# medhini/audio-video-textures

Measured on AMD Instinct MI355X. Metric: clip-windows/sec encoded + N×N transition build, N=4096; HBM GB/s achieved, higher is better.
Workload: dtype f16x3

## Files before the change

audio-video-textures_amd/csrc/conv_x3.hip:

```cpp
#include <stdlib.h>

#include <type_traits>

#include "avt_common.h"
#include "conv_args.h"
#include "split_planes.h"

#ifdef AVT_CONV_STAMP
#define AVT_STAMP_FN avt_debug_stamps_x3
namespace {
#include "../../tools/diag/conv_stamp.h"
}
#ifndef AVT_DBG_CONST
#define AVT_DBG_CONST 0
#endif
#define DBG_SKIP(bit) (((AVT_DBG_CONST) & (bit)) != 0)
#ifdef AVT_STAMP_EPI
#define KSTAMP(i) STAMP(0)
#define EPI_STAMP(i) STAMP(i)
#else
#define KSTAMP(i) STAMP(i)
#define EPI_STAMP(i)
#endif
#else
// ... 762 lines not shown
            }
          }
          float* of = reinterpret_cast<float*>(a.out) + o;
          typedef float f32x4n __attribute__((ext_vector_type(4)));
          __builtin_nontemporal_store(f32x4n{x[0], x[1], x[2], x[3]}, reinterpret_cast<f32x4n*>(of));
          __builtin_nontemporal_store(f32x4n{x[4], x[5], x[6], x[7]}, reinterpret_cast<f32x4n*>(of + 4));
        } else {
          uint4 oh, ol;
          avt::split8<F16>(x, oh, ol);
          *reinterpret_cast<uint4*>(a.out + o) = oh;
          *reinterpret_cast<uint4*>(a.out_lo + o) = ol;
        }
      }
    }
    EPI_STAMP(3);
    __syncthreads();
    EPI_STAMP(4);
  }
  if constexpr (IO32) {
    if (a.stat_part) {
      float* red = reinterpret_cast<float*>(lds);
      const int tr = tid / CPR, cc = tid % CPR;
#pragma unroll
      for (int e = 0; e < 8; ++e) {
        red[(tr * 2 + 0) * BN + cc * 8 + e] = st_s[e];
        red[(tr * 2 + 1) * BN + cc * 8 + e] = st_q[e];
      }
      __syncthreads();
      stat_fold_store<BN, NTHR>(a, red, NTHR / CPR, tm, n0, tid);
    }
  }
  STAMP_END();
}

template <bool F16, bool IO32 = false, bool OUT32 = IO32>
int launch_x3_xl(ConvArgs& a, hipStream_t st) {
  if (a.stat_part) a.stat_tpg = (a.stat_mg + 255) / 256;
  const int tiles_m = a.stat_part ? a.stat_groups * a.stat_tpg : (a.M + 255) / 256;
  a.tiles_n = (a.Cout + 255) / 256;
  a.nblk = tiles_m * a.tiles_n;
  constexpr int lds_max = 2 * 4 * 256 * 64 + kMaxTabSteps * 64 + 2 * 256 * 4;
  const int lds_bytes = lds_max;
  a.cf_ofs = lds_max - 2 * 256 * 4;
  static const hipError_t e = hipFuncSetAttribute(reinterpret_cast<const void*>(conv_x3_xl_kernel<F16, IO32, OUT32>),
                                                  hipFuncAttributeMaxDynamicSharedMemorySize, lds_max);
  if (e != hipSuccess) {
    avt::set_error("avt_conv3d_igemm_x3: hipFuncSetAttribute(%d B LDS): %s", lds_max, hipGetErrorString(e));
    return AVT_ERR_LAUNCH;
  }
  hipLaunchKernelGGL((conv_x3_xl_kernel<F16, IO32, OUT32>), dim3((unsigned)a.nblk), dim3(512), lds_bytes, st, a);
  return avt::check_launch("avt_conv3d_igemm_x3");
}

template <int BM, int BN, int WTM, bool F16, bool IO32 = false, bool BST = false>
int launch_x3(ConvArgs& a, hipStream_t st) {
  if (a.stat_part) a.stat_tpg = (a.stat_mg + BM - 1) / BM;
  const int tiles_m = a.stat_part ? a.stat_groups * a.stat_tpg : (a.M + BM - 1) / BM;
  a.tiles_n = (a.Cout + BN - 1) / BN;
  a.nblk = tiles_m * a.tiles_n;
  constexpr int epi_bytes = BM * (BN * 4 + 16);
  constexpr int opnd_max = 2 * (BM + BN) * LSTR + kMaxTabSteps * 64;
  constexpr int lds_max = (opnd_max > epi_bytes ? opnd_max : epi_bytes) + 2 * BN * 4;
  const int tab_bytes = (a.nk <= kMaxTabSteps ? a.nk : 0) * 64;
  int lds_bytes = 2 * (BM + BN) * LSTR + tab_bytes;
  if (lds_bytes < epi_bytes) lds_bytes = epi_bytes;
  a.cf_ofs = lds_bytes;
  lds_bytes += 2 * BN * 4;
  static const hipError_t e = hipFuncSetAttribute(reinterpret_cast<const void*>(conv_x3_kernel<BM, BN, WTM, F16, IO32, BST>),
                                                  hipFuncAttributeMaxDynamicSharedMemorySize, lds_max);
  if (e != hipSuccess) {
    avt::set_error("avt_conv3d_igemm_x3: hipFuncSetAttribute(%d B LDS): %s", lds_max, hipGetErrorString(e));
    return AVT_ERR_LAUNCH;
  }
  hipLaunchKernelGGL((conv_x3_kernel<BM, BN, WTM, F16, IO32, BST>), dim3((unsigned)a.nblk), dim3(256), lds_bytes, st, a);
  return avt::check_launch("avt_conv3d_igemm_x3");
}

}

extern "C" int avt_conv3d_igemm_x3_xl_picked(int cout, int k, int m) {
  return (cout % 256 == 0 && k >= 256 && k <= kMaxTabSteps * 64 && m >= 256 * 64) ? 1 : 0;
}

static int igemm_x3_impl(const void* in_hi, const void* in_lo, const void* wt_hi, const void* wt_lo,
                         const float* bias, const void* res_hi, const void* res_lo, void* out_hi, void* out_lo,
                         const int32_t* ktab, int batch, int t, int h, int w, int cin, int cout, int kt, int kh,
                         int kw, int st, int sh, int sw, int pt, int ph, int pw, int to, int ho, int wo, int ldi,
                         int ldo, int ldr, int relu, int out_row_stride, int out_h, int out_w, int plane_dtype,
                         const float* wscale, void* stream, int wblk) {
  AVT_REQUIRE(plane_dtype == AVT_X3_BF16 || plane_dtype == AVT_X3_F16, "avt_conv3d_igemm_x3: plane_dtype must be 0 (bf16) or 1 (fp16)");
  AVT_REQUIRE(!wscale || avt::aligned16(wscale), "avt_conv3d_igemm_x3: wscale must be 16-byte aligned");
  AVT_REQUIRE(in_lo && wt_lo && out_lo && (!res_hi == !res_lo), "avt_conv3d_igemm_x3: every tensor needs both planes");
  AVT_REQUIRE(avt::aligned16(in_lo) && avt::aligned16(wt_lo) && avt::aligned16(out_lo) && (!res_lo || avt::aligned16(res_lo)),
              "avt_conv3d_igemm_x3: pointers must be 16-byte aligned");
  ConvArgs a;
  const int rc = conv_args_fill(a, "avt_conv3d_igemm_x3", in_hi, wt_hi, bias, res_hi, out_hi, ktab, batch, t, h, w, cin, cout,
                                kt, kh, kw, st, sh, sw, pt, ph, pw, to, ho, wo, ldi, ldo, ldr, relu, out_row_stride, out_h,
                                out_w);
  if (rc != AVT_OK) return rc;
  a.in_lo = static_cast<const uint16_t*>(in_lo);
  a.wt_lo = static_cast<const uint16_t*>(wt_lo);
  a.res_lo = static_cast<const uint16_t*>(res_lo);
  a.out_lo = static_cast<uint16_t*>(out_lo);
  a.wscale = wscale;
  a.wfrag = nullptr;
  a.nup = 0;
  a.wblk = wblk;
  hipStream_t s = static_cast<hipStream_t>(stream);
  AVT_REQUIRE(!wblk || (avt_conv3d_igemm_x3_xl_picked(cout, a.K, a.M) && a.K % 32 == 0),
              "avt_conv3d_igemm_x3_wblk: K-blocked weights are the 256 x 256 tile's (avt_conv3d_igemm_x3_xl_picked, K %% 32 == 0)");
  if (avt_conv3d_igemm_x3_xl_picked(cout, a.K, a.M))
    return plane_dtype == AVT_X3_F16 ? launch_x3_xl<true>(a, s) : launch_x3_xl<false>(a, s);
  if (plane_dtype == AVT_X3_F16) {
    if (cout <= 32) return launch_x3<128, 32, 32, true>(a, s);
    if (cout <= 64) return launch_x3<128, 64, 64, true>(a, s);
    return launch_x3<128, 128, 64, true>(a, s);
  }
  if (cout <= 32) return launch_x3<128, 32, 32, false>(a, s);
  if (cout <= 64) return launch_x3<128, 64, 64, false>(a, s);
  return launch_x3<128, 128, 64, false>(a, s);
}

extern "C" int avt_conv3d_igemm_x3(const void* in_hi, const void* in_lo, const void* wt_hi, const void* wt_lo,
                                   const float* bias, const void* res_hi, const void* res_lo, void* out_hi, void* out_lo,
                                   const int32_t* ktab, int batch, int t, int h, int w, int cin, int cout, int kt, int kh,
                                   int kw, int st, int sh, int sw, int pt, int ph, int pw, int to, int ho, int wo, int ldi,
                                   int ldo, int ldr, int relu, int out_row_stride, int out_h, int out_w, int plane_dtype,
                                   const float* wscale, void* stream) {
  return igemm_x3_impl(in_hi, in_lo, wt_hi, wt_lo, bias, res_hi, res_lo, out_hi, out_lo, ktab, batch, t, h, w, cin, cout, kt, kh, kw,
                       st, sh, sw, pt, ph, pw, to, ho, wo, ldi, ldo, ldr, relu, out_row_stride, out_h, out_w, plane_dtype, wscale,
                       stream, 0);
}

extern "C" int avt_conv3d_igemm_x3_wblk(const void* in_hi, const void* in_lo, const void* wt_hi, const void* wt_lo,
                                        const float* bias, const void* res_hi, const void* res_lo, void* out_hi, void* out_lo,
                                        const int32_t* ktab, int batch, int t, int h, int w, int cin, int cout, int kt, int kh,
                                        int kw, int st, int sh, int sw, int pt, int ph, int pw, int to, int ho, int wo, int ldi,
                                        int ldo, int ldr, int relu, int out_row_stride, int out_h, int out_w, int plane_dtype,
                                        const float* wscale, void* stream) {
  return igemm_x3_impl(in_hi, in_lo, wt_hi, wt_lo, bias, res_hi, res_lo, out_hi, out_lo, ktab, batch, t, h, w, cin, cout, kt, kh, kw,
                       st, sh, sw, pt, ph, pw, to, ho, wo, ldi, ldo, ldr, relu, out_row_stride, out_h, out_w, plane_dtype, wscale,
                       stream, 1);
}

extern "C" int avt_gemm_nt_x3_f32out(const void* a_hi, const void* a_lo, int lda, const void* b_hi, const void* b_lo, float* out, int64_t ldo,
                                     int m, int n, int k, float divisor, const int32_t* ktab, int plane_dtype, void* stream) {
  AVT_REQUIRE(plane_dtype == AVT_X3_BF16 || plane_dtype == AVT_X3_F16, "avt_gemm_nt_x3_f32out: plane_dtype must be 0 (bf16) or 1 (fp16)");
  AVT_REQUIRE(a_lo && b_lo && avt::aligned16(a_lo) && avt::aligned16(b_lo) && divisor != 0.0f, "avt_gemm_nt_x3_f32out: both planes, divisor != 0");
  AVT_REQUIRE(m > 0 && n % 256 == 0 && k % 32 == 0 && k >= 256 && k <= kMaxTabSteps * 64 && ldo >= n && ldo % 4 == 0 && ldo < (1ll << 31),
              "avt_gemm_nt_x3_f32out: n %% 256 == 0, 256 <= k <= %d in multiples of 32 (got m %d n %d k %d)", kMaxTabSteps * 64, m, n, k);
  ConvArgs a;
  const int rc = conv_args_fill(a, "avt_gemm_nt_x3_f32out", a_hi, b_hi, nullptr, nullptr, out, ktab, 1, 1, 1, m, k, n, 1, 1, 1, 1, 1, 1, 0, 0, 0,
                                0, 0, 0, lda, 8 * (int)((ldo + 7) / 8), 0, 0, 1, 0, 0);
  if (rc != AVT_OK) return rc;
  a.ldo = (int)ldo;
  a.in_lo = static_cast<const uint16_t*>(a_lo);
  a.wt_lo = static_cast<const uint16_t*>(b_lo);
  a.res_lo = nullptr;
  a.out_lo = nullptr;
  a.wscale = nullptr;
  a.wfrag = nullptr;
  a.nup = 0;
  a.wblk = 0;
  a.odiv = divisor;
  hipStream_t s = static_cast<hipStream_t>(stream);
  return plane_dtype == AVT_X3_F16 ? launch_x3_xl<true, false, true>(a, s) : launch_x3_xl<false, false, true>(a, s);
}

static int g_io32_small = 1;
static int io32_tile_rows(int cout, int k, int64_t m) {
  if (k % 32 == 0 && m < (1ll << 31) && avt_conv3d_igemm_x3_xl_picked(cout, k, (int)m) && m >= 256 * 256) return 256;
  if (g_io32_small && cout > 64 && ((m + 127) / 128) * ((cout + 127) / 128) < 512) return 64;
  return 128;
}

extern "C" int avt_conv_x3_set_small_tile(int on) {
  const int was = g_io32_small;
  g_io32_small = on ? 1 : 0;
  return was;
}

static int igemm_x3_f32_impl(const float* in, const void* wt_hi, const void* wt_lo, const float* wscale, const float* add,
                             float* out, const int32_t* ktab, int batch, int t, int h, int w, int cin, int cout, int kt, int kh,
                             int kw, int st, int sh, int sw, int pt, int ph, int pw, int to, int ho, int wo, int ldi, int ldo, int lda,
                             int out_row_stride, int out_h, int out_w, int plane_dtype, void* stream, double* stat_part = nullptr,
                             int stat_groups = 0, int stat_c = 0, const ConvArgs* bst = nullptr) {
  AVT_REQUIRE(plane_dtype == AVT_X3_BF16 || plane_dtype == AVT_X3_F16, "avt_conv3d_igemm_x3_f32: plane_dtype must be 0 (bf16) or 1 (fp16)");
  AVT_REQUIRE(wt_lo && avt::aligned16(wt_lo) && (!wscale || avt::aligned16(wscale)), "avt_conv3d_igemm_x3_f32: weight planes / wscale NULL or unaligned");
  AVT_REQUIRE((int64_t)batch * t * h * w * ldi < (1ll << 30) - 64, "avt_conv3d_igemm_x3_f32: input too large for 32-bit byte offsets");
  ConvArgs a;
  const int rc = conv_args_fill(a, "avt_conv3d_igemm_x3_f32", in, wt_hi, nullptr, add, out, ktab, batch, t, h, w, cin, cout, kt, kh, kw,
                                st, sh, sw, pt, ph, pw, to, ho, wo, ldi, ldo, add ? lda : 0, 0, out_row_stride, out_h, out_w);
  if (rc != AVT_OK) return rc;
  a.in_bytes *= 2u;
  a.in_lo = nullptr;
  a.wt_lo = static_cast<const uint16_t*>(wt_lo);
  a.res_lo = nullptr;
  a.out_lo = nullptr;
  a.wscale = wscale;
  a.wfrag = nullptr;
  a.nup = 0;
  a.wblk = 0;
  if (stat_part) {
// ... 99 lines not shown
```

audio-video-textures_amd/fused_slowfast.py:

```python
import torch
import torch.nn as nn

from . import ops
from ._lib import AvtError


_FUSE_BLOCK = 1
_C33 = 1
_CHAIN = 1
_CHAIN_MAXN = 512
_FUSE_KCAT = 1
_XB = 1
_FUSE_SCAT = 1
_FUSE_TCHUNK = 0
_FUSE_BLOCK_X3 = 1
_FUSE_TCHUNK_X3 = 0
_CHAIN_X3 = 1
_WBLK_X3 = 1
_STEM_FM_X3 = 1
_C33_X3 = 1
_RES2_X3 = 1
_PW_X3 = 1
_STEM_LDS = 1
_STEM_POOL = 1
_PW_X3_SKIP = {(512, 128), (320, 128)}
_LATERAL_X3 = {(32, 64)}
_STEM_MERGE = 1
_KW1_CAP = 32

PROFILER = None


class Act:

    __slots__ = ("buf", "dims", "c0", "C", "lo")

    def __init__(self, buf, dims, c0=0, C=None, lo=None):
        self.buf, self.dims, self.c0, self.lo = buf, dims, c0, lo
        self.C = buf.shape[1] - c0 if C is None else C

    @property
    def ptr(self):
        return self.buf.data_ptr() + 2 * self.c0

    @property
    def ptrs(self):
        return (self.buf.data_ptr() + 2 * self.c0, self.lo.data_ptr() + 2 * self.c0)

    @property
    def ld(self):
        return self.buf.shape[1]

    def float(self, plane_dtype=None):
        if self.lo is None:
            return self.buf[:, self.c0 : self.c0 + self.C].float()
        dt = torch.float16 if plane_dtype == ops.X3_F16 else torch.bfloat16
        sl = slice(self.c0, self.c0 + self.C)
        return self.buf.view(dt)[:, sl].float() + self.lo.view(dt)[:, sl].float()


def new_act(m, c, dims, device, x3=False):
    buf = torch.empty((m, c), dtype=torch.bfloat16, device=device)
    return Act(buf, dims, lo=torch.empty_like(buf) if x3 else None)


def split_planes(w, plane_dtype):
    w = w.detach().float()
    dt = torch.float16 if plane_dtype == ops.X3_F16 else torch.bfloat16
    hi = w.to(dt)
    lo = (w - hi.float()).to(dt)
    return hi.view(torch.bfloat16).contiguous(), lo.view(torch.bfloat16).contiguous()


def fold_bn(conv, bn):
    w = conv.weight.detach().float()
    if bn is not None:
        scale = bn.weight.detach().float() / torch.sqrt(bn.running_var.detach().float() + bn.eps)
        bias = bn.bias.detach().float() - bn.running_mean.detach().float() * scale
        w = w * scale.view(-1, 1, 1, 1, 1)
    else:
        bias = conv.bias.detach().float() if conv.bias is not None else torch.zeros(w.shape[0])
    return w, bias


def group_weights_w(w, g):
    cout, cin, kt, kh, kw = w.shape
    r = kw // 2
    rg = -(-r // g)
    kwg = 1 + 2 * rg
    wg = torch.zeros((g, cout, g, cin, kt, kh, kwg))
    for po in range(g):
        for dg in range(kwg):
            for pi in range(g):
                dw = g * (dg - rg) + pi - po + r
                if 0 <= dw < kw:
                    wg[po, :, pi, :, :, :, dg] = w[:, :, :, :, dw]
    return wg.reshape(g * cout, g * cin, kt, kh, kwg), rg
# ... 614 lines not shown
                return self._chain(m, self.c.cin, self.c, sc, chain, m.dims, y=out, x2=x2)
            return self.c(m, out=out, res=sc, relu=True)
        if (self.fused is not None and out is None and x.c0 == 0 and x.ld == x.C and
                ops.bottleneck_fused_supported(x.C, x.dims[3])):
            b, t, h, w = x.dims
            y = Act(torch.empty((b * t * h * w, x.C), dtype=torch.bfloat16, device=self.dev), x.dims)

            def launch():
                ops.bottleneck_fused(x.ptr, y.ptr, self.fused, b, t, h, w, x.C, tchunk=_FUSE_TCHUNK or (16 if w >= 56 else 32))

            if PROFILER is None:
                launch()
            else:
                m = b * t * h * w
                fl = m * (self.a.alg_flops_per_row + self.b.alg_flops_per_row + self.c.alg_flops_per_row)
                PROFILER("bottleneck_kernel", launch, fl, 2.0 * (2 * m * x.C))
            return y
        if (self.fused_first is not None and out is None and x.c0 == 0 and x.ld == x.C and
                ops.bottleneck_first_supported(x.C, self.c.cout, x.dims[3]) and x.dims[2] % self.b.stride[1] == 0):
            b, t, h, w = x.dims
            st = self.b.stride[1]
            od = (b, t, h // st, w // st)
            mo = od[0] * od[1] * od[2] * od[3]
            y = Act(torch.empty((mo, self.c.cout), dtype=torch.bfloat16, device=self.dev), od)

            def launch():
                ops.bottleneck_first(x.ptr, y.ptr, self.fused_first, b, t, h, w, x.C, self.c.cout,
                                     tchunk=_FUSE_TCHUNK or (16 if w >= 56 else 32))

            if PROFILER is None:
                launch()
            else:
                m = b * t * h * w
                fl = (m * self.a.alg_flops_per_row +
                      mo * (self.b.alg_flops_per_row + self.c.alg_flops_per_row + self.b1.alg_flops_per_row))
                PROFILER("bottleneck_kernel", launch, fl, 2.0 * (m * x.C + mo * self.c.cout))
            return y
        sc = self.b1(x) if self.b1 is not None else x
        return self.c(self._b(self.a(x)), out=out, res=sc, relu=True)


class _BlockX3:

    def __init__(self, blk, device, x3):
        self.b1 = FusedConv(blk.branch1, blk.branch1_bn, False, device, x3=x3) if hasattr(blk, "branch1") else None
        t = blk.branch2
        self.a = FusedConv(t.a, t.a_bn, True, device, x3=x3)
        self.b = FusedConv(t.b, t.b_bn, True, device, x3=x3)
        self.c = FusedConv(t.c, t.c_bn, True, device, x3=x3)
        self.x3, self.dev = x3, device
        self.fused = None
        shape_ok = (self.a.kernel == (3, 1, 1) and self.b.kernel == (1, 3, 3) and self.c.kernel == (1, 1, 1) and
                    self.a.stride == (1, 1, 1) and self.a.cout <= 32)
        s1 = self.b.stride == (1, 1, 1)
        ident = s1 and self.b1 is None and self.c.cout == self.a.cin and self.c.cout in (32, 64, 128)
        first8 = (s1 and self.b1 is not None and self.a.cin == 8 and self.c.cout == 32 and self.b1.kernel == (1, 1, 1) and
                  self.b1.stride == (1, 1, 1))
        strided = (self.b1 is not None and self.b.stride == (1, 2, 2) and self.b1.stride == (1, 2, 2) and
                   self.b1.kernel == (1, 1, 1) and self.a.cin in (32, 64) and self.c.cout == 2 * self.a.cin)
        self.st = 2 if strided else 1
        if _FUSE_BLOCK_X3 and shape_ok and (ident or first8 or strided):
            (wa, ba), (wb, bb), (wc, bc) = self.a._folded, self.b._folded, self.c._folded
            self.fused = pack_bottleneck_x3(wa, ba, wb, bb, wc, bc, x3, device,
                                            shortcut=self.b1._folded if (first8 or strided) else None)
        self.c33 = None
        if (_C33_X3 and self.fused is None and self.b.kernel == (1, 3, 3) and self.b.stride == (1, 1, 1) and
                self.b._folded is not None and ops.conv33_x3_supported(self.b.cin, self.b.cout)):
            self.c33 = pack_c33_x3(self.b._folded[0], self.b._folded[1], x3, device)
        self.res2 = None
        if (_RES2_X3 and x3 == ops.X3_F16 and self.fused is None and self.b1 is None and self.a.kernel == (1, 1, 1) and
                self.a.stride == (1, 1, 1) and self.b.kernel == (1, 3, 3) and self.b.stride == (1, 1, 1) and self.c.kernel == (1, 1, 1) and
                self.c.stride == (1, 1, 1) and self.a.cin == self.c.cout and all(v._folded is not None for v in (self.a, self.b, self.c)) and
                ops.res2_x3_supported(self.c.cout, self.a.cout, 56)):
            (wa, ba), (wb, bb), (wc, bc) = self.a._folded, self.b._folded, self.c._folded
            self.res2 = pack_res2_x3(wa, ba, wb, bb, wc, bc, x3, device)
        self.ccat, self.extra = None, 0
        if (_FUSE_KCAT and self.b1 is not None and self.fused is None and self.a.kernel == (1, 1, 1) and
                self.c.kernel == (1, 1, 1) and self.b1.kernel == (1, 1, 1) and self.a.stride == (1, 1, 1) and
                self.b.stride == (1, 1, 1) and self.b1.stride == (1, 1, 1) and self.c.stride == (1, 1, 1)):
            (wsc, bsc), (wc, bc) = self.b1._folded, self.c._folded
            self.ccat = FusedConv(None, None, True, device, folded=(torch.cat([wsc, wc], 1), bc + bsc, (1, 1, 1), (0, 0, 0)), x3=x3)
            self.ccat.alg_flops_per_row = self.c.alg_flops_per_row + self.b1.alg_flops_per_row
            self.extra = self.c.cin

    def can_chain(self, nxt):
        if self.res2 is not None or (nxt is not None and nxt.res2 is not None):
            return False
        return (_CHAIN_X3 and nxt is not None and self.b1 is None and self.fused is None and nxt.fused is None and
                getattr(self.c, "pw", None) is not None and getattr(nxt.a, "pw", None) is not None and nxt.ccat is None and
                nxt.a.cin == self.c.cout and ops.pw_chain_x3_supported(self.c.cin, self.c.cout, nxt.a.cout))

    def __call__(self, x, out=None, chain=None, a_pre=None):
        if chain is not None or a_pre is not None:
            m = self._b(a_pre if a_pre is not None else self.a(x))
            sc = self.b1(x) if self.b1 is not None else x
            if chain is None:
                return self.c(m, out=out, res=sc, relu=True)
            rows = m.dims[0] * m.dims[1] * m.dims[2] * m.dims[3]
            y = out if out is not None else new_act(rows, self.c.cout, m.dims, self.dev, True)
            z = new_act(rows, chain.a.cout, m.dims, self.dev, True)

            def launch():
                ops.pw_chain_x3(m.ptrs, m.ld, self.c.cin, self.c.pw, self.c.bias, self.c.wscale, sc.ptrs, sc.ld, y.ptrs, y.ld,
                                self.c.cout, True, chain.a.pw, chain.a.bias, chain.a.wscale, z.ptrs, z.ld, chain.a.cout, rows,
                                self.x3)

            if PROFILER is None:
                launch()
            else:
                PROFILER("pw_chain_x3_kernel", launch, rows * (self.c.alg_flops_per_row + chain.a.alg_flops_per_row),
                         4.0 * rows * (self.c.cin + 2 * self.c.cout + chain.a.cout))
            return y, z
        if (self.res2 is not None and chain is None and a_pre is None and x.lo is not None and x.C == self.a.cin and
                ops.res2_x3_supported(self.c.cout, self.a.cout, x.dims[3])):
            b, t, h, w = x.dims
            rows = b * t * h * w
            y = out if out is not None else new_act(rows, self.c.cout, x.dims, self.dev, True)

            def launch():
                ops.res2_x3(x.ptrs, x.ld, y.ptrs, y.ld, self.res2, b, t, h, w, self.x3)

            if PROFILER is None:
                launch()
            else:
                fl = rows * (self.a.alg_flops_per_row + self.b.alg_flops_per_row + self.c.alg_flops_per_row)
                PROFILER("res2_x3_kernel", launch, fl, 4.0 * rows * 2 * self.c.cout)
            return y
        if (self.fused is not None and out is None and x.c0 == 0 and x.ld == x.C and
                ops.bneck_x3_supported(x.C, self.c.cout, x.dims[3]) and x.dims[2] % self.st == 0):
            b, t, h, w = x.dims
            od = (b, t, h // self.st, w // self.st)
            mo = od[0] * od[1] * od[2] * od[3]
            y = new_act(mo, self.c.cout, od, self.dev, True)

            def launch():
                ops.bneck_x3(x.ptrs, y.ptrs, self.fused, b, t, h, w, x.C, self.c.cout, self.x3,
                             tchunk=_FUSE_TCHUNK_X3 or (11 if w == 14 else 8))

            if PROFILER is None:
                launch()
            else:
                m = b * t * h * w
                fl = m * self.a.alg_flops_per_row + mo * (self.b.alg_flops_per_row + self.c.alg_flops_per_row +
                                                          (self.b1.alg_flops_per_row if self.b1 is not None else 0.0))
                PROFILER("bneck_x3_kernel", launch, fl, 4.0 * (m * x.C + mo * self.c.cout))
            return y
        if self.ccat is not None and x.c0 == 0 and x.lo is not None and x.ld >= x.C + self.extra and x.C == self.a.cin:
            self._b(self.a(x), out=Act(x.buf, x.dims, x.C, self.extra, lo=x.lo))
            return self.ccat(Act(x.buf, x.dims, 0, x.C + self.extra, lo=x.lo), out=out)
        sc = self.b1(x) if self.b1 is not None else x
        return self.c(self._b(self.a(x)), out=out, res=sc, relu=True)

    def _b(self, m, out=None):
        if self.c33 is None:
            return self.b(m, out=out)
        b, t, h, w = m.dims
        if out is None:
            out = new_act(b * t * h * w, self.b.cout, m.dims, self.dev, True)

        def launch():
            ops.conv33_x3(m.ptrs, self.c33, out.ptrs, b, t, h, w, m.ld, out.ld, self.x3, relu=True)

        if PROFILER is None:
            launch()
        else:
            rows = b * t * h * w
            PROFILER("conv33_x3_kernel", launch, rows * self.b.alg_flops_per_row, 4.0 * rows * 2 * self.b.cout)
        return out


PRECISIONS = {"bf16": None, "bf16x3": ops.X3_BF16, "f16x3": ops.X3_F16}


class SlowFastMFMA(nn.Module):

# ... 90 lines not shown
        nf = clip.table_frames if table else b * t
        kt = conv.kernel[0]
        per_frame = table and kt == 1 and conv.tgroup == 1 and conv.stride[0] == 1
        sb, st_ = (nf, 1) if per_frame else (b, t)
        x = Act(clip.hi.view(nf * h * (w // 2), 8), (sb, st_, h, w // 2), lo=clip.lo.view(nf * h * (w // 2), 8))
        pool_idx = clip.idx.reshape(-1) if per_frame else None
        merged = None
        if (table and lds_path and _STEM_MERGE and conv.frames_per_tile == 2 and getattr(conv, "wg", None) is not None and
                clip.start is not None and t == 32):
            merged = merged_stem_taps(conv, clip.win_len, self.dev)
        if merged is not None:
            od = conv.out_dims(x.dims)
            m_out = od[0] * od[1] * od[2] * od[3]
            y = new_act(m_out, conv.cout, od, self.dev, True)
            src = merged["src"]
            taps = torch.where(src.unsqueeze(0) >= 0, clip.start.view(-1, 1, 1) + src.unsqueeze(0), src.unsqueeze(0)).contiguous()

            def launch():
                ops.stem_conv_x3_merged(x.ptrs, merged["wt_hi"], merged["wt_lo"], merged["bias"], merged["wscale"], y.ptrs, b, t, h,
                                        w // 2, conv.cout, conv.kernel[0], conv.stride[0], conv.pad[0], self.x3, taps,
                                        merged["tiles"], merged["ktm"], nf, relu=True)

            if PROFILER is None:
                launch()
            else:
                PROFILER("stem_kernel<x3>", launch, m_out * conv.alg_flops_per_row,
                         4.0 * (x.buf.numel() + m_out * conv.cout) + conv.wt.numel() * 4)
        elif lds_path:
            od = conv.out_dims(x.dims)
            m_out = od[0] * od[1] * od[2] * od[3]
            y = new_act(m_out, conv.cout, od, self.dev, True)

            def launch():
                ops.stem_conv_x3(x.ptrs, conv.wt_lds, conv.wt_lds_lo, conv.bias, conv.wscale, y.ptrs, sb, st_, h, w // 2,
                                 conv.cout, conv.kernel[0], conv.stride[0], conv.pad[0], self.x3, relu=True,
                                 frames_per_tile=conv.frames_per_tile, frame_idx=clip.idx if (table and not per_frame) else None,
                                 table_frames=nf if (table and not per_frame) else 0)

            if PROFILER is None:
                launch()
            else:
                PROFILER("stem_kernel<x3>", launch, m_out * conv.alg_flops_per_row,
                         4.0 * (x.buf.numel() + m_out * conv.cout) + conv.wt.numel() * 4)
        else:
            y = conv(x)
        _, tg, h2, w2 = y.dims
        pd = (b, t, (h2 - 1) // 2 + 1, (w2 - 1) // 2 + 1)
        cf = conv.frame_channels
        if out is None:
            out = new_act(pd[0] * pd[1] * pd[2] * pd[3], cf, pd, self.dev, True)
        if per_frame:
            ops.maxpool_hw3s2_x3(y.ptrs, out.ptrs, b * t, h2, w2, conv.cout, y.ld, out.ld, self.x3, frame_idx=pool_idx)
        else:
            ops.maxpool_hw3s2_x3(y.ptrs, out.ptrs, b * tg, h2, w2, conv.cout, y.ld, out.ld, self.x3, tgroup=conv.tgroup)
        return out, pd

    @torch.no_grad()
    def _forward_x3(self, slow, fast):
        b = slow.shape[0]
        f_act, df = self._stem_x3(self.stem_f, fast)
        cs, cf = self.stem_s.frame_channels, self.stem_f.frame_channels
        hs, ws = (slow.shape[2] // 2 - 1) // 2 + 1, (slow.shape[3] // 2 - 1) // 2 + 1
        ds = (b, slow.shape[1], hs, ws)
        extra = getattr(self.stages[0][0][0], "extra", 0)
        cat = new_act(ds[0] * ds[1] * ds[2] * ds[3], cs + 2 * cf + extra, ds, self.dev, True)
        sl = lambda a, c0, c: Act(a.buf, a.dims, c0, c, lo=a.lo)
        self._stem_x3(self.stem_s, slow, out=sl(cat, 0, cs))
        self.fuse[0](f_act, out=sl(cat, cs, 2 * cf))
        s_act = sl(cat, 0, cs + 2 * cf)
        for k, (slow_blocks, fast_blocks) in enumerate(self.stages):
            for blk in fast_blocks:
                f_act = blk(f_act)
            last = k == len(self.stages) - 1
            pre = None
            for i, blk in enumerate(slow_blocks):
                nxt = slow_blocks[i + 1] if i + 1 < len(slow_blocks) else None
                if blk.can_chain(nxt):
                    s_act, pre = blk(s_act, chain=nxt, a_pre=pre)
                    continue
                a_pre, pre = pre, None
                if i == len(slow_blocks) - 1 and not last:
                    od = blk.b.out_dims(blk.a.out_dims(s_act.dims))
                    cs, cf = blk.c.cout, f_act.C
                    cat = new_act(od[0] * od[1] * od[2] * od[3], cs + 2 * cf, od, self.dev, True)
                    blk(s_act, out=sl(cat, 0, cs), a_pre=a_pre)
                    self.fuse[k + 1](f_act, out=sl(cat, cs, 2 * cf))
                    s_act = cat
                else:
                    s_act = blk(s_act, a_pre=a_pre)
        emb = torch.empty((b, s_act.C + f_act.C), dtype=torch.float32, device=self.dev)
        ops.mean_positions_x3(s_act.ptrs, b, s_act.buf.shape[0] // b, s_act.C, s_act.ld, emb, 0, self.x3)
        ops.mean_positions_x3(f_act.ptrs, b, f_act.buf.shape[0] // b, f_act.C, f_act.ld, emb, s_act.C, self.x3)
        return emb

    @torch.no_grad()
    def forward_ndhwc4(self, slow, fast):
        if self.x3 is not None:
            return self._forward_x3(slow, fast)
        b = slow.shape[0]
        f_act, df = self._stem(self.stem_f, fast)
        cs, cf = self.stem_s.frame_channels, self.stem_f.frame_channels
        hs, ws = (slow.shape[2] // 2 - 1) // 2 + 1, (slow.shape[3] // 2 - 1) // 2 + 1
        ds = (b, slow.shape[1], hs, ws)
        extra = self.stages[0][0][0].extra
        sbuf = torch.empty((ds[0] * ds[1] * ds[2] * ds[3], cs + 2 * cf + extra), dtype=torch.bfloat16, device=self.dev)
        self._stem(self.stem_s, slow, out=Act(sbuf, ds, 0, cs))
        self.fuse[0](f_act, out=Act(sbuf, ds, cs, 2 * cf))
        s_act = Act(sbuf, ds, 0, cs + 2 * cf)
        pre = None
        for k, (slow_blocks, fast_blocks) in enumerate(self.stages):
            for blk in fast_blocks:
                f_act = blk(f_act)
            last = k == len(self.stages) - 1
            for i, blk in enumerate(slow_blocks):
                nxt = slow_blocks[i + 1] if i + 1 < len(slow_blocks) else None
                if blk.can_chain(nxt, s_act):
                    s_act, pre = blk(s_act, chain=nxt, a_pre=pre)
                    continue
                a_pre, pre = pre, None
                if i == len(slow_blocks) - 1 and not last:
                    od = blk.b.out_dims(blk.a.out_dims(s_act.dims))
                    cs, cf = blk.c.cout, f_act.C
                    nxt0 = self.stages[k + 1][0][0]
                    sbuf = torch.empty((od[0] * od[1] * od[2] * od[3], cs + 2 * cf + nxt0.extra), dtype=torch.bfloat16,
                                       device=self.dev)
                    if blk.can_chain(nxt0, s_act):
                        self.fuse[k + 1](f_act, out=Act(sbuf, od, cs, 2 * cf))
                        _, pre = blk(s_act, out=Act(sbuf, od, 0, cs), chain=nxt0, a_pre=a_pre, x2=Act(sbuf, od, cs, 2 * cf))
                    else:
                        blk(s_act, out=Act(sbuf, od, 0, cs), a_pre=a_pre)
                        self.fuse[k + 1](f_act, out=Act(sbuf, od, cs, 2 * cf))
                    s_act = Act(sbuf, od, 0, cs + 2 * cf)
                else:
                    s_act = blk(s_act, a_pre=a_pre)
        emb = torch.empty((b, s_act.C + f_act.C), dtype=torch.float32, device=self.dev)
        ops.mean_positions(s_act.ptr, b, s_act.buf.shape[0] // b, s_act.C, s_act.ld, emb, 0)
        ops.mean_positions(f_act.ptr, b, f_act.buf.shape[0] // b, f_act.C, f_act.ld, emb, s_act.C)
        return emb
```

audio-video-textures_amd/ops.py:

```python
import ctypes as C

import numpy as np
import torch

from . import _lib

SIM_BF16, SIM_BF16X3, SIM_F32 = 0, 1, 2
_PREC = {"bf16": SIM_BF16, "bf16x3": SIM_BF16X3, "f32": SIM_F32}
FAST_T, SLOW_T, SLOTS = 32, 8, 40


def _dev(t, name, dtype=None, contiguous=True):
    if not isinstance(t, torch.Tensor) or not t.is_cuda:
        raise _lib.AvtError("%s must be a device (HIP) tensor; the hot path has no CPU fallback" % name)
    if dtype is not None and t.dtype != dtype:
        raise _lib.AvtError("%s must be %s, got %s" % (name, dtype, t.dtype))
    if contiguous and not t.is_contiguous():
        raise _lib.AvtError("%s must be contiguous" % name)
    return t


def _p(t):
    return None if t is None else C.c_void_p(t.data_ptr())

# ... 694 lines not shown
def maxpool_hw2s2_x3(x_ptrs, out_ptrs, bt, h, w, c, ldi, ldo, plane_dtype):
    _lib.check(_lib.lib().avt_maxpool_hw2s2_ndhwc_x3(C.c_void_p(x_ptrs[0]), C.c_void_p(x_ptrs[1]), C.c_void_p(out_ptrs[0]),
                                                     C.c_void_p(out_ptrs[1]), int(bt), int(h), int(w), int(c), int(ldi),
                                                     int(ldo), int(plane_dtype), _stream()), "avt_maxpool_hw2s2_ndhwc_x3")


def maxpool3d_k3s2_x3(x_ptrs, out_ptrs, batch, t, h, w, c, ldi, ldo, plane_dtype):
    _lib.check(_lib.lib().avt_maxpool3d_k3s2_ndhwc_x3(C.c_void_p(x_ptrs[0]), C.c_void_p(x_ptrs[1]), C.c_void_p(out_ptrs[0]),
                                                      C.c_void_p(out_ptrs[1]), int(batch), int(t), int(h), int(w), int(c),
                                                      int(ldi), int(ldo), int(plane_dtype), _stream()), "avt_maxpool3d_k3s2_ndhwc_x3")


def mean_positions_x3(x_ptrs, batch, p, c, ldi, out, col0, plane_dtype):
    _dev(out, "out", torch.float32)
    _lib.check(_lib.lib().avt_mean_positions_x3(C.c_void_p(x_ptrs[0]), C.c_void_p(x_ptrs[1]), int(batch), int(p), int(c),
                                                int(ldi), C.c_void_p(out.data_ptr() + 4 * int(col0)), int(out.shape[1]),
                                                int(plane_dtype), _stream()), "avt_mean_positions_x3")


def maxpool_hw3s2(x_ptr, out_ptr, bt, h, w, c, ldi, ldo, tgroup=1):
    _lib.check(_lib.lib().avt_maxpool_hw3s2_ndhwc_bf16(C.c_void_p(x_ptr), C.c_void_p(out_ptr), int(bt), int(h), int(w),
                                                       int(c), int(ldi), int(ldo), int(tgroup), _stream()),
               "avt_maxpool_hw3s2_ndhwc_bf16")


def stem_conv_supported(h, pw, cout):
    return bool(_lib.lib().avt_stem_conv_supported(int(h), int(pw), int(cout)))


def stem_conv(x_ptr, wt, bias, out_ptr, batch, t, h, pw, cout, kt, st, pt, relu=True):
    _dev(wt, "wt", torch.bfloat16)
    _dev(bias, "bias", torch.float32)
    _lib.check(_lib.lib().avt_stem_conv_bf16(C.c_void_p(x_ptr), _p(wt), _p(bias), C.c_void_p(out_ptr), int(batch), int(t),
                                             int(h), int(pw), int(cout), int(kt), int(st), int(pt), int(bool(relu)),
                                             _stream()), "avt_stem_conv_bf16")


def stem_conv_pool(x_ptr, wt, bias, out_ptr, batch, t, h, pw, cout, kt, st, pt, tgroup, ldo):
    _dev(wt, "wt", torch.bfloat16)
    _dev(bias, "bias", torch.float32)
    _lib.check(_lib.lib().avt_stem_conv_pool_bf16(C.c_void_p(x_ptr), _p(wt), _p(bias), C.c_void_p(out_ptr), int(batch),
                                                  int(t), int(h), int(pw), int(cout), int(kt), int(st), int(pt),
                                                  int(tgroup), int(ldo), _stream()), "avt_stem_conv_pool_bf16")


def bottleneck_fused_supported(c, w):
    return bool(_lib.lib().avt_bottleneck_fused_supported(int(c), int(w)))


def bottleneck_fused(x_ptr, out_ptr, packed, batch, t, h, w, c, tchunk=8):
    wa, ba, wb, bb, wc, bc = packed
    _lib.check(_lib.lib().avt_bottleneck_fused_bf16(C.c_void_p(x_ptr), C.c_void_p(out_ptr), _p(wa), _p(ba), _p(wb), _p(bb),
                                                    _p(wc), _p(bc), int(batch), int(t), int(h), int(w), int(c),
                                                    int(tchunk), _stream()), "avt_bottleneck_fused_bf16")


def conv3d_igemm_x3_xl_picked(cout, k, m):
    return bool(_lib.lib().avt_conv3d_igemm_x3_xl_picked(int(cout), int(k), int(m)))


def conv33_x3_supported(cin, cout):
    return bool(_lib.lib().avt_conv33_x3_supported(int(cin), int(cout)))


def conv33_x3(x_ptrs, packed, out_ptrs, batch, t, h, w, ldi, ldo, plane_dtype, relu=True):
    wfrag, coef = packed
    _dev(wfrag, "wfrag", torch.bfloat16)
    _dev(coef, "coef", torch.float32)
    _lib.check(_lib.lib().avt_conv33_x3(C.c_void_p(x_ptrs[0]), C.c_void_p(x_ptrs[1]), _p(wfrag), _p(coef), C.c_void_p(out_ptrs[0]),
                                        C.c_void_p(out_ptrs[1]), int(batch), int(t), int(h), int(w), int(ldi), int(ldo),
                                        int(bool(relu)), int(plane_dtype), _stream()), "avt_conv33_x3")


def res2_x3_supported(c, cm, w):
    return bool(_lib.lib().avt_res2_x3_supported(int(c), int(cm), int(w)))


def res2_x3(x_ptrs, ldi, out_ptrs, ldo, packed, batch, t, h, w, plane_dtype):
    wfrag, coef = packed
    _dev(wfrag, "wfrag", torch.bfloat16)
    _dev(coef, "coef", torch.float32)
    if wfrag.numel() * 2 != _lib.lib().avt_res2_x3_wfrag_bytes():
        raise _lib.AvtError("res2_x3: wfrag holds %d bytes, the kernel streams %d" % (wfrag.numel() * 2, _lib.lib().avt_res2_x3_wfrag_bytes()))
    _lib.check(_lib.lib().avt_res2_x3(C.c_void_p(x_ptrs[0]), C.c_void_p(x_ptrs[1]), C.c_void_p(out_ptrs[0]), C.c_void_p(out_ptrs[1]),
                                      _p(wfrag), _p(coef), int(batch), int(t), int(h), int(w), int(ldi), int(ldo), int(plane_dtype),
                                      _stream()), "avt_res2_x3")


def bneck_x3_supported(cin, c, w):
    return bool(_lib.lib().avt_bneck_x3_supported(int(cin), int(c), int(w)))


def bneck_x3(x_ptrs, out_ptrs, packed, batch, t, h, w, cin, c, plane_dtype, tchunk=16):
    wfrag, coef = packed
    _dev(wfrag, "wfrag", torch.bfloat16)
    _dev(coef, "coef", torch.float32)
    _lib.check(_lib.lib().avt_bneck_x3(C.c_void_p(x_ptrs[0]), C.c_void_p(x_ptrs[1]), C.c_void_p(out_ptrs[0]),
                                       C.c_void_p(out_ptrs[1]), _p(wfrag), _p(coef), int(batch), int(t), int(h), int(w),
                                       int(cin), int(c), int(tchunk), int(plane_dtype), _stream()), "avt_bneck_x3")


def mean_positions(x_ptr, batch, p, c, ldi, out, col0=0):
    _dev(out, "out", torch.float32)
    _lib.check(_lib.lib().avt_mean_positions_bf16(C.c_void_p(x_ptr), int(batch), int(p), int(c), int(ldi),
                                                  C.c_void_p(out.data_ptr() + 4 * int(col0)), int(out.shape[1]), _stream()),
               "avt_mean_positions_bf16")


def bottleneck_first_supported(cin, c, w):
    return bool(_lib.lib().avt_bottleneck_first_supported(int(cin), int(c), int(w)))


def bottleneck_first(x_ptr, out_ptr, packed, batch, t, h, w, cin, c, tchunk=8):
    wa, ba, wb, bb, wc, bc, wsc = packed
    _lib.check(_lib.lib().avt_bottleneck_first_bf16(C.c_void_p(x_ptr), C.c_void_p(out_ptr), _p(wa), _p(ba), _p(wb), _p(bb),
                                                    _p(wc), _p(wsc), _p(bc), int(batch), int(t), int(h), int(w), int(cin),
                                                    int(c), int(tchunk), _stream()), "avt_bottleneck_first_bf16")


def conv33_c64_supported(cin, cout, w):
    return bool(_lib.lib().avt_conv33_c64_supported(int(cin), int(cout), int(w)))


def conv33_c64(x_ptr, wb, bias, out_ptr, batch, t, h, w, ldo, relu=True):
    _dev(wb, "wb", torch.bfloat16)
    _dev(bias, "bias", torch.float32)
    _lib.check(_lib.lib().avt_conv33_c64_bf16(C.c_void_p(x_ptr), _p(wb), _p(bias), C.c_void_p(out_ptr), int(batch), int(t),
                                              int(h), int(w), int(ldo), int(bool(relu)), _stream()), "avt_conv33_c64_bf16")


def pw_chain_supported(k1, n1, n2, has_res, k2x=0):
    return bool(_lib.lib().avt_pw_chain_supported(int(k1), int(n1), int(n2), int(bool(has_res)), int(k2x)))


def pw_chain(x1_ptr, ldx, k1, w1, b1, res_ptr, ldr, y_ptr, ldy, n1, w2, b2, z_ptr, ldz, n2, m, x2_ptr=0, ldx2=0, k2x=0):
    _dev(w1, "w1", torch.bfloat16)
    _dev(w2, "w2", torch.bfloat16)
    _dev(b1, "b1", torch.float32)
    _dev(b2, "b2", torch.float32)
    _lib.check(_lib.lib().avt_pw_chain_bf16(C.c_void_p(x1_ptr), int(ldx), int(k1), _p(w1), _p(b1),
                                            C.c_void_p(res_ptr) if res_ptr else None, int(ldr), C.c_void_p(y_ptr), int(ldy),
                                            int(n1), C.c_void_p(x2_ptr) if x2_ptr else None, int(ldx2), int(k2x), _p(w2),
                                            _p(b2), C.c_void_p(z_ptr), int(ldz), int(n2), int(m), _stream()),
               "avt_pw_chain_bf16")


def maxpool_hw2s2(x_ptr, out_ptr, bt, h, w, c, ldi, ldo):
    _lib.check(_lib.lib().avt_maxpool_hw2s2_ndhwc_bf16(C.c_void_p(x_ptr), C.c_void_p(out_ptr), int(bt), int(h), int(w),
                                                       int(c), int(ldi), int(ldo), _stream()),
               "avt_maxpool_hw2s2_ndhwc_bf16")


def pairwise_l2(x):
    _dev(x, "x", torch.float32)
    n, d = x.shape
    out = torch.empty((n, n), dtype=torch.float32, device=x.device)
    _lib.check(_lib.lib().avt_pairwise_l2_f32(_p(x), int(n), int(d), _p(out), _stream()), "avt_pairwise_l2_f32")
    return out


def diag_filter(d1, w):
    _dev(d1, "d1", torch.float32)
    _dev(w, "w", torch.float32)
    n, fs = d1.shape[0], int(w.numel())
    out = torch.empty((n - fs + 1, n - fs + 1), dtype=torch.float32, device=d1.device)
    _lib.check(_lib.lib().avt_diag_filter_f32(_p(d1), int(n), _p(w), fs, _p(out), _stream()), "avt_diag_filter_f32")
    return out


# ... 107 lines not shown
```

Before: 1441.

## Fuse strided shortcut and expand convs in x3 bottlenecks; split oversized launches

Adds a fused 'scat' path for x3 bottleneck blocks with a strided 1x1 shortcut. The 3x3 conv output is written next to the block input in a wider buffer, and the shortcut conv and the final 1x1 expand conv run as one concatenated-K conv with stride 2. This removes a separate shortcut launch and its intermediate read and write. The stage-transition concat buffer is widened to hold the extra channels, and chaining is disabled for such blocks. Separately, igemm_x3 and res2_x3 split very large inputs into frame or batch ranges so offsets stay within 32-bit limits, which adds host-side launch loops.

New measurement: 1475, median of 6. 2.4% higher.

```diff
diff --git a/audio-video-textures_amd/csrc/conv_x3.hip b/audio-video-textures_amd/csrc/conv_x3.hip
--- a/audio-video-textures_amd/csrc/conv_x3.hip
+++ b/audio-video-textures_amd/csrc/conv_x3.hip
@@ -868,12 +868,12 @@
   return (cout % 256 == 0 && k >= 256 && k <= kMaxTabSteps * 64 && m >= 256 * 64) ? 1 : 0;
 }
 
-static int igemm_x3_impl(const void* in_hi, const void* in_lo, const void* wt_hi, const void* wt_lo,
-                         const float* bias, const void* res_hi, const void* res_lo, void* out_hi, void* out_lo,
-                         const int32_t* ktab, int batch, int t, int h, int w, int cin, int cout, int kt, int kh,
-                         int kw, int st, int sh, int sw, int pt, int ph, int pw, int to, int ho, int wo, int ldi,
-                         int ldo, int ldr, int relu, int out_row_stride, int out_h, int out_w, int plane_dtype,
-                         const float* wscale, void* stream, int wblk) {
+static int igemm_x3_one(const void* in_hi, const void* in_lo, const void* wt_hi, const void* wt_lo,
+                        const float* bias, const void* res_hi, const void* res_lo, void* out_hi, void* out_lo,
+                        const int32_t* ktab, int batch, int t, int h, int w, int cin, int cout, int kt, int kh,
+                        int kw, int st, int sh, int sw, int pt, int ph, int pw, int to, int ho, int wo, int ldi,
+                        int ldo, int ldr, int relu, int out_row_stride, int out_h, int out_w, int plane_dtype,
+                        const float* wscale, void* stream, int wblk, int xl) {
   AVT_REQUIRE(plane_dtype == AVT_X3_BF16 || plane_dtype == AVT_X3_F16, "avt_conv3d_igemm_x3: plane_dtype must be 0 (bf16) or 1 (fp16)");
   AVT_REQUIRE(!wscale || avt::aligned16(wscale), "avt_conv3d_igemm_x3: wscale must be 16-byte aligned");
   AVT_REQUIRE(in_lo && wt_lo && out_lo && (!res_hi == !res_lo), "avt_conv3d_igemm_x3: every tensor needs both planes");
@@ -893,10 +893,9 @@
   a.nup = 0;
   a.wblk = wblk;
   hipStream_t s = static_cast<hipStream_t>(stream);
-  AVT_REQUIRE(!wblk || (avt_conv3d_igemm_x3_xl_picked(cout, a.K, a.M) && a.K % 32 == 0),
+  AVT_REQUIRE(!wblk || (xl && a.K % 32 == 0),
               "avt_conv3d_igemm_x3_wblk: K-blocked weights are the 256 x 256 tile's (avt_conv3d_igemm_x3_xl_picked, K %% 32 == 0)");
-  if (avt_conv3d_igemm_x3_xl_picked(cout, a.K, a.M))
-    return plane_dtype == AVT_X3_F16 ? launch_x3_xl<true>(a, s) : launch_x3_xl<false>(a, s);
+  if (xl) return plane_dtype == AVT_X3_F16 ? launch_x3_xl<true>(a, s) : launch_x3_xl<false>(a, s);
   if (plane_dtype == AVT_X3_F16) {
     if (cout <= 32) return launch_x3<128, 32, 32, true>(a, s);
     if (cout <= 64) return launch_x3<128, 64, 64, true>(a, s);
@@ -905,6 +904,56 @@
   if (cout <= 32) return launch_x3<128, 32, 32, false>(a, s);
   if (cout <= 64) return launch_x3<128, 64, 64, false>(a, s);
   return launch_x3<128, 128, 64, false>(a, s);
+}
+
+static int igemm_x3_impl(const void* in_hi, const void* in_lo, const void* wt_hi, const void* wt_lo,
+                         const float* bias, const void* res_hi, const void* res_lo, void* out_hi, void* out_lo,
+                         const int32_t* ktab, int batch, int t, int h, int w, int cin, int cout, int kt, int kh,
+                         int kw, int st, int sh, int sw, int pt, int ph, int pw, int to, int ho, int wo, int ldi,
+                         int ldo, int ldr, int relu, int out_row_stride, int out_h, int out_w, int plane_dtype,
+                         const float* wscale, void* stream, int wblk) {
+  constexpr int64_t kMaxPlane = (1ll << 31) - 64;
+  const bool sane = batch > 0 && t > 0 && h > 0 && w > 0 && ldi > 0 && ldo > 0 && cin > 0 && cout > 0 && kt >= 1 && kh >= 1 && kw >= 1 &&
+                    st >= 1 && sh >= 1 && sw >= 1 && ph >= 0 && pw >= 0 && ho >= 0 && wo >= 0 && out_row_stride >= 1 && out_h >= 0 && out_w >= 0;
+  const int64_t frame = sane ? (int64_t)h * w * ldi : 0, frames = sane ? (int64_t)batch * t : 0;
+  if (!sane || frame * frames < kMaxPlane || kt != 1 || st != 1 || pt != 0 || (to != 0 && to != t)) {
+    const int64_t k_all = (int64_t)kt * kh * kw * cin;
+    int xl = 0;
+    if (sane && k_all < (1ll << 31)) {
+      const int64_t fho = ho > 0 ? ho : (h + 2 * ph - kh) / sh + 1, fwo = wo > 0 ? wo : (w + 2 * pw - kw) / sw + 1;
+      const int64_t fto = to > 0 ? to : (t + 2 * pt - kt) / st + 1;
+      const int64_t m = (int64_t)batch * fto * fho * fwo;
+      xl = (m > 0 && m < (1ll << 31)) ? avt_conv3d_igemm_x3_xl_picked(cout, (int)k_all, (int)m) : 0;
+    }
+    return igemm_x3_one(in_hi, in_lo, wt_hi, wt_lo, bias, res_hi, res_lo, out_hi, out_lo, ktab, batch, t, h, w, cin, cout, kt, kh, kw, st,
+                        sh, sw, pt, ph, pw, to, ho, wo, ldi, ldo, ldr, relu, out_row_stride, out_h, out_w, plane_dtype, wscale, stream, wblk,
+                        xl);
+  }
+  AVT_REQUIRE(frame < kMaxPlane, "avt_conv3d_igemm_x3: one frame's input plane (%d x %d x %d elements) is too large for 32-bit offsets", h, w,
+              ldi);
+  AVT_REQUIRE(in_hi && in_lo && out_hi && out_lo && (!res_hi == !res_lo), "avt_conv3d_igemm_x3: every tensor needs both planes");
+  const int fho = ho > 0 ? ho : (h + 2 * ph - kh) / sh + 1, fwo = wo > 0 ? wo : (w + 2 * pw - kw) / sw + 1;
+  AVT_REQUIRE(fho > 0 && fwo > 0, "avt_conv3d_igemm_x3: bad output extent");
+  const bool remap = out_row_stride > 1 || (out_h > 0 && out_w > 0);
+  const int64_t m_all = frames * fho * fwo;
+  const int64_t orows = remap ? (int64_t)out_h * out_w : (int64_t)fho * fwo;
+  AVT_REQUIRE(m_all < (1ll << 31) && frames * orows < (1ll << 31) && (int64_t)kh * kw * cin < (1ll << 31),
+              "avt_conv3d_igemm_x3: tensor too large for 32-bit rows");
+  const int xl = avt_conv3d_igemm_x3_xl_picked(cout, kh * kw * cin, (int)m_all);
+  const int64_t fmax = kMaxPlane / frame;
+  const int64_t nrange = (frames + fmax - 1) / fmax;
+  const int64_t per = (frames + nrange - 1) / nrange;
+  for (int64_t f0 = 0; f0 < frames; f0 += per) {
+    const int nf = (int)((frames - f0 < per) ? frames - f0 : per);
+    const int64_t io = f0 * frame, oo = f0 * orows * ldo, ro = f0 * fho * fwo * ldr;
+    auto adv = [](const void* p, int64_t e) { return p ? static_cast<const void*>(static_cast<const uint16_t*>(p) + e) : nullptr; };
+    const int rc = igemm_x3_one(adv(in_hi, io), adv(in_lo, io), wt_hi, wt_lo, bias, adv(res_hi, ro), adv(res_lo, ro),
+                                const_cast<void*>(adv(out_hi, oo)), const_cast<void*>(adv(out_lo, oo)), ktab, nf, 1, h, w, cin, cout, kt, kh,
+                                kw, st, sh, sw, pt, ph, pw, to ? 1 : 0, ho, wo, ldi, ldo, ldr, relu, out_row_stride, out_h, out_w,
+                                plane_dtype, wscale, stream, wblk, xl);
+    if (rc != AVT_OK) return rc;
+  }
+  return AVT_OK;
 }
 
 extern "C" int avt_conv3d_igemm_x3(const void* in_hi, const void* in_lo, const void* wt_hi, const void* wt_lo,
diff --git a/audio-video-textures_amd/fused_slowfast.py b/audio-video-textures_amd/fused_slowfast.py
--- a/audio-video-textures_amd/fused_slowfast.py
+++ b/audio-video-textures_amd/fused_slowfast.py
@@ -13,6 +13,8 @@
 _XB = 1
 _FUSE_SCAT = 1
 _FUSE_TCHUNK = 0
+_FUSE_SCAT_X3 = 1
+_SCAT_X3_SKIP = set()
 _FUSE_BLOCK_X3 = 1
 _FUSE_TCHUNK_X3 = 0
 _CHAIN_X3 = 1
@@ -793,15 +795,34 @@
             self.ccat = FusedConv(None, None, True, device, folded=(torch.cat([wsc, wc], 1), bc + bsc, (1, 1, 1), (0, 0, 0)), x3=x3)
             self.ccat.alg_flops_per_row = self.c.alg_flops_per_row + self.b1.alg_flops_per_row
             self.extra = self.c.cin
+        self.scat = None
+        if (_FUSE_SCAT_X3 and self.b1 is not None and self.fused is None and self.ccat is None and
+                self.c.kernel == (1, 1, 1) and self.b1.kernel == (1, 1, 1) and self.b.kernel == (1, 3, 3) and
+                self.b.stride == (1, 2, 2) and self.b1.stride == (1, 2, 2) and self.a.stride == (1, 1, 1) and
+                self.c.stride == (1, 1, 1) and self.a.kernel[1:] == (1, 1) and self.b1._folded is not None and
+                (self.a.cin, self.c.cout) not in _SCAT_X3_SKIP):
+            (wsc, bsc), (wc, bc) = self.b1._folded, self.c._folded
+            self.scat = FusedConv(None, None, True, device, folded=(torch.cat([wsc, wc], 1), bc + bsc, (1, 2, 2), (0, 0, 0)), x3=x3)
+            self.scat.alg_flops_per_row = self.c.alg_flops_per_row + self.b1.alg_flops_per_row
+            self.extra = self.c.cin
+
+    def _scat_ok(self, x):
+        return (self.scat is not None and x.c0 == 0 and x.lo is not None and x.ld >= x.C + self.extra and x.C == self.a.cin and
+                x.dims[2] % 2 == 0 and x.dims[3] % 2 == 0)
 
     def can_chain(self, nxt):
         if self.res2 is not None or (nxt is not None and nxt.res2 is not None):
+            return False
+        if self.scat is not None or (nxt is not None and nxt.scat is not None):
             return False
         return (_CHAIN_X3 and nxt is not None and self.b1 is None and self.fused is None and nxt.fused is None and
                 getattr(self.c, "pw", None) is not None and getattr(nxt.a, "pw", None) is not None and nxt.ccat is None and
                 nxt.a.cin == self.c.cout and ops.pw_chain_x3_supported(self.c.cin, self.c.cout, nxt.a.cout))
 
     def __call__(self, x, out=None, chain=None, a_pre=None):
+        if chain is None and a_pre is None and self._scat_ok(x):
+            self.b(self.a(x), out=Act(x.buf, x.dims, x.C, self.extra, lo=x.lo), out_rows=(2, x.dims[2], x.dims[3]))
+            return self.scat(Act(x.buf, x.dims, 0, x.C + self.extra, lo=x.lo), out=out)
         if chain is not None or a_pre is not None:
             m = self._b(a_pre if a_pre is not None else self.a(x))
             sc = self.b1(x) if self.b1 is not None else x
@@ -1058,10 +1079,11 @@
                 if i == len(slow_blocks) - 1 and not last:
                     od = blk.b.out_dims(blk.a.out_dims(s_act.dims))
                     cs, cf = blk.c.cout, f_act.C
-                    cat = new_act(od[0] * od[1] * od[2] * od[3], cs + 2 * cf, od, self.dev, True)
+                    extra = self.stages[k + 1][0][0].extra if (od[2] % 2 == 0 and od[3] % 2 == 0) else 0
+                    cat = new_act(od[0] * od[1] * od[2] * od[3], cs + 2 * cf + extra, od, self.dev, True)
                     blk(s_act, out=sl(cat, 0, cs), a_pre=a_pre)
                     self.fuse[k + 1](f_act, out=sl(cat, cs, 2 * cf))
-                    s_act = cat
+                    s_act = sl(cat, 0, cs + 2 * cf)
                 else:
                     s_act = blk(s_act, a_pre=a_pre)
         emb = torch.empty((b, s_act.C + f_act.C), dtype=torch.float32, device=self.dev)
diff --git a/audio-video-textures_amd/ops.py b/audio-video-textures_amd/ops.py
--- a/audio-video-textures_amd/ops.py
+++ b/audio-video-textures_amd/ops.py
@@ -800,9 +800,15 @@
     _dev(coef, "coef", torch.float32)
     if wfrag.numel() * 2 != _lib.lib().avt_res2_x3_wfrag_bytes():
         raise _lib.AvtError("res2_x3: wfrag holds %d bytes, the kernel streams %d" % (wfrag.numel() * 2, _lib.lib().avt_res2_x3_wfrag_bytes()))
-    _lib.check(_lib.lib().avt_res2_x3(C.c_void_p(x_ptrs[0]), C.c_void_p(x_ptrs[1]), C.c_void_p(out_ptrs[0]), C.c_void_p(out_ptrs[1]),
-                                      _p(wfrag), _p(coef), int(batch), int(t), int(h), int(w), int(ldi), int(ldo), int(plane_dtype),
-                                      _stream()), "avt_res2_x3")
+    clip_bytes = int(t) * int(h) * int(w) * max(int(ldi), int(ldo)) * 2
+    ranges = -(-int(batch) * clip_bytes // ((1 << 32) - 65)) if clip_bytes > 0 else 1
+    per = -(-int(batch) // max(ranges, 1))
+    for b0 in range(0, int(batch), max(per, 1)):
+        nb = min(per, int(batch) - b0)
+        xo, oo = b0 * t * h * w * int(ldi) * 2, b0 * t * h * w * int(ldo) * 2
+        _lib.check(_lib.lib().avt_res2_x3(C.c_void_p(x_ptrs[0] + xo), C.c_void_p(x_ptrs[1] + xo), C.c_void_p(out_ptrs[0] + oo),
+                                          C.c_void_p(out_ptrs[1] + oo), _p(wfrag), _p(coef), nb, int(t), int(h), int(w), int(ldi), int(ldo),
+                                          int(plane_dtype), _stream()), "avt_res2_x3")
 
 
 def bneck_x3_supported(cin, c, w):
```
